# thalesfm/differentiable-renderer

Measured on AMD Instinct MI355X. Metric: Mray/s (fwd+bwd), Cornell 512x512 @64spp depth 8, higher is better.
Workload: dtype f32; 1 GPU; config 3: Cornell 512x512, 64 spp, depth 8, fwd + radiative backprop w.r.t. the albedos; scene 'cornell' (cornell box of render.cpp:26-59) 512x512, 64 spp per GPU, depth 8 (-b 8 -p 1), fwd + radiative-backprop gradients of 4 parameters; program=builtin, parallelism=1 GPU, gpu_max_hw_queues=4 (set by this script before the HIP runtime started)

## Files before the change

differentiable-renderer_amd/csrc/drt_path.h:

```cpp
#pragma once

#include "drt_kernels.h"

#define DRT_DRAW_TABLE (3 * DRT_MAX_DEPTH + 8)

struct PathArgs {
    int32_t W, H, spp;
    int32_t shard, n_shards, band;
    uint32_t Pb, p0, Sb, s0, spr, n_ranges, n_groups;
    int32_t min_bounces, depth_cap, cap_is_roulette, cap_draws;
    uint32_t rr_threshold, seed, rng_stream;
    uint32_t regen_min;
    uint32_t shade_min, descend_min;
    int32_t gimg_param;
    uint32_t gen_rows, gen_clog2;
    uint32_t hist_lds, hist_stride;
    uint32_t gimg_row, pad_gen;
    unsigned long long hist_ovf;
    double p_rr, inv_p_rr;
    double eye[3], fwd[3], right[3], up[3];
    double tan_half, aspect, inv_W, inv_H;
    float p_rr_f, inv_p_rr_f;
    float eye_f[3], fwd_f[3], right_f[3], up_f[3], cs_step_f, ct_step_f;
};
// ... 335 lines not shown
template <typename R>
__device__ inline void gen_zero(GenBlock<R>& gb)
{
    typedef typename GenAcc<R>::T GT;
    for (uint32_t i = threadIdx.x; i < (DRT_BLOCK / DRT_WAVE) * DRT_GEN_TABLE; i += DRT_BLOCK)
        (&gb.table[0][0])[i] = GT(0);
}
template <typename R, int NC, typename SL>
__device__ inline void gen_begin(GenBlock<R>& gb, const SL& lds, const DevScene<R>* __restrict__ sc, const PathArgs& a, uint32_t* hist,
                                 uint32_t* hist_ovf, Tangents<R, DRT_NP_ANY, NC>& tg)
{
    stage_gen(gb.gl, lds, sc);
    tg.gl = &gb.gl;
    tg.hist = hist + threadIdx.x;
    tg.hist_ovf = hist_ovf + (size_t)blockIdx.x * DRT_BLOCK + threadIdx.x;
    tg.gsum = mk<R>(R(0), R(0), R(0));
    tg.gimg_row = a.gimg_row;
    tg.hist_lds = a.hist_lds;
    tg.hist_stride = a.hist_stride;
    tg.clog2 = a.gen_clog2;
    tg.table = &gb.table[threadIdx.x / DRT_WAVE][threadIdx.x & ((1u << a.gen_clog2) - 1u)];
    tg.acc = nullptr;
    tg.new_path();
}
template <typename R>
__device__ inline void gen_finish(const GenBlock<R>& gb, const PathArgs& a, double* __restrict__ gpart)
{
    __syncthreads();
    const uint32_t copies = 1u << a.gen_clog2;
    for (uint32_t r = threadIdx.x; r < a.gen_rows; r += DRT_BLOCK) {
        double v = 0;
        for (int ww = 0; ww < DRT_BLOCK / DRT_WAVE; ++ww)
            for (uint32_t c = 0; c < copies; ++c)
                v += (double)gb.table[ww][(r << a.gen_clog2) + c];
        gpart[(size_t)blockIdx.x * a.gen_rows + r] = v;
    }
}

#define DRT_NC_ROLES(nc, colour_mask, emission_mask) ((int)(nc) | (int)(colour_mask) << 8 | (int)(emission_mask) << 16)
#define DRT_NC_OF(ncr) ((int)(ncr) & 0xFF)
#define DRT_ROLES_OF(ncr) ((int)(ncr) >> 8)
#define DRT_ROLES_CORNELL DRT_ROLES_OF(DRT_NC_ROLES(0, 0x7, 0x8))
template <int NP, int NC, int ROLES>
struct PathRoles {
    static constexpr int all = NP > 0 ? (1 << NP) - 1 : 0;
    static constexpr int colm = ROLES ? (ROLES & 0xFF) & ((1 << NC) - 1) : (1 << NC) - 1;
    static constexpr int emitm = ROLES ? (ROLES >> 8) & all : all;
    static __device__ constexpr bool colour(int p) { return (colm >> p) & 1; }
    static __device__ constexpr bool emission(int p) { return (emitm >> p) & 1; }
    static __device__ constexpr bool only_emission(int p) { return emitm == (1 << p); }
};

template <typename R, int NP, int NC, bool LOSS = false, typename SL = PathSceneLds<R>, int ROLES = 0>
__device__ inline void add_emission(const SL& lds, const TangentLds<R>& tl, const R* __restrict__ params, uint32_t eid, R inv_pk,
                                    V3<R> T, V3<R> g, V3<R>& L, Tangents<R, NP, NC>& tg)
{
    const V3<R> E = load_param<R, (NP != 0)>(lds, params, (int)eid) * inv_pk;
    V3<R> Tr = T;
    if (NC > 0 || NP == DRT_NP_ANY || NP == DRT_NP_TANGENT)
        Tr = mk<R>((tg.zc & 0xFFu) ? R(0) : T.x, (tg.zc & 0xFF00u) ? R(0) : T.y, (tg.zc & 0xFF0000u) ? R(0) : T.z);
    L = L + Tr * E;
    if constexpr (NP == DRT_NP_TANGENT) {
        const R* vd = tg.dl->dir + (eid < DRT_PATH_LDS_PARAMS ? eid : 0u) * 3u;
        const V3<R> Ed = mk<R>(vd[0], vd[1], vd[2]) * inv_pk;
        const V3<R> d0 = mk<R>(fma_r(E.x, tg.S.x, Ed.x), fma_r(E.y, tg.S.y, Ed.y), fma_r(E.z, tg.S.z, Ed.z));
        const V3<R> d1 = E * tg.Z;
        const uint32_t zx = tg.zc & 0xFFu, zy = tg.zc & 0xFF00u, zz = tg.zc & 0xFF0000u;
        tg.dL = mk<R>(fma_r(T.x, zx == 0u ? d0.x : (zx == 0x1u ? d1.x : R(0)), tg.dL.x),
                      fma_r(T.y, zy == 0u ? d0.y : (zy == 0x100u ? d1.y : R(0)), tg.dL.y),
                      fma_r(T.z, zz == 0u ? d0.z : (zz == 0x10000u ? d1.z : R(0)), tg.dL.z));
    } else
    if constexpr (NP == DRT_NP_ANY) {
        if (LOSS)
            g = mk<R>(R(2) * (L.x - g.x), R(2) * (L.y - g.y), R(2) * (L.z - g.z));
        const V3<R> gE = g * E;
        const uint32_t ebits = pid_unpack(tg.gl->invc[eid < DRT_PATH_LDS_PARAMS ? eid : 0][3]);
        if ((ebits & 0xFFFFu) != DRT_SLOT_NONE && eid < DRT_PATH_LDS_PARAMS)
            tg.add(ebits & 0xFFFFu, g * Tr * inv_pk);
        const V3<R> TgE = Tr * gE;
        const V3<R> U = mk<R>((tg.zc & 0xFFu) == 0x1u ? T.x * gE.x : R(0), (tg.zc & 0xFF00u) == 0x100u ? T.y * gE.y : R(0),
                              (tg.zc & 0xFF0000u) == 0x10000u ? T.z * gE.z : R(0));
        const uint32_t nw = tg.nv >> 2;
        for (uint32_t w = 0; wave_any(w < nw); ++w)
            tg.add_word(w < nw ? tg.load_word(w) : 0xFFFFFFFFu, TgE, U);
        tg.add_word(tg.cur, TgE, U);
    } else
    if constexpr (NP > 0) {
        if (NC > 0)
            asm volatile("" ::: "memory");
        if (LOSS)
            g = mk<R>(R(2) * (L.x - g.x), R(2) * (L.y - g.y), R(2) * (L.z - g.z));
        const V3<R> gE = g * E, gT = g * Tr * inv_pk;
#pragma unroll
        for (int p = 0; p < NP; ++p) {
            typedef PathRoles<NP, NC, ROLES> RL;
            const bool is_colour = (RL::colm >> p) & 1, is_emission = (RL::emitm >> p) & 1;
            if (ROLES != 0 && !is_colour && !is_emission)
                continue;
            const bool own = (ROLES != 0 && RL::emitm == (1 << p)) || eid == (uint32_t)p;
            const V3<R> ap = tg.acc_get(p);
            V3<R> a0 = mk<R>(ap.x + (own ? gT.x : R(0)), ap.y + (own ? gT.y : R(0)), ap.z + (own ? gT.z : R(0)));
            if (ROLES != 0 && !is_emission)
                a0 = ap;
            if (is_colour) {
                const uint32_t n = (tg.cnt[p >> 2] >> (8 * (p & 3))) & 0xFFu;
                const R nf = (R)(int)n;
                V3<R> dT = mk<R>(Tr.x * (nf * tl.invc[p][0]), Tr.y * (nf * tl.invc[p][1]), Tr.z * (nf * tl.invc[p][2]));
                const uint32_t zb = __builtin_amdgcn_readfirstlane(tl.inc[p][3]);
                if (zb) {
                    const bool one = n == 1u;
                    if (zb & 1u) dT.x = (one && (tg.zc & 0xFFu) == 0x1u) ? T.x : R(0);
                    if (zb & 2u) dT.y = (one && (tg.zc & 0xFF00u) == 0x100u) ? T.y : R(0);
                    if (zb & 4u) dT.z = (one && (tg.zc & 0xFF0000u) == 0x10000u) ? T.z : R(0);
                }
                tg.acc_set(p, mk<R>(fma_r(dT.x, gE.x, a0.x), fma_r(dT.y, gE.y, a0.y), fma_r(dT.z, gE.z, a0.z)));
            } else
                tg.acc_set(p, a0);
        }
    }
}

template <typename R>
struct CameraLane {
    R cs0, ct0;
};

template <typename R>
struct PathVertex {
    V3<R> P, nrm, d;
    uint32_t ids;
    int material;
    bool hit, scattered;
};

template <typename R, bool SPEC, int NP, int NC, typename SG, bool FREEZE_BY_ROW = false>
__device__ inline void path_bounce(const PathArgs& a, const PathSceneLds<R>& lds, const TangentLds<R>& tl, const DevScene<R>* __restrict__ sc,
                                   const R* __restrict__ params, const ProgRecs<SG::n, R>& recs, uint32_t key,
                                   R pk, R inv_pk, uint32_t n_theta, bool next_rr, bool next_cap, bool live, V3<R> g,
                                   typename Q4<R>::T& ra, typename Q2<R>::T& rb, V3<R>& T, V3<R>& L, Tangents<R, NP, NC>& tg,
                                   bool& alive, bool& capped, bool& on_light, uint32_t& light, PathVertex<R>* vo = nullptr,
                                   bool last = false, const float* __restrict__ seed_px = nullptr, const uint32_t* ih = nullptr)
{
    auto draw = [&](uint32_t n) { return ih ? drt_rng_combine(ih[n], key) : rng_draw(a.rng_stream, key, n); };
    const HitRec<R> h = path_closest_hit<SG>(sc, recs, ra, rb);
    const bool hit = live && h.prim >= 0;
    const int prim = h.prim >= 0 ? h.prim : 0;
    const V3<R> o = mk<R>(ra.x, ra.y, ra.z);
    const V3<R> d = mk<R>(ra.w, rb.x, rb.y);
    const V3<R> P = o + d * h.t;
    const DevShape<R>& sh = lds.sc.shapes[prim];
    const uint32_t ids = (uint32_t)sh.pad;
    const uint32_t cid = ids & 0xFFFFu, eid = ids >> 16;
    const bool has_bxdf = cid != DRT_ID_NONE, emits = hit && eid != DRT_ID_NONE;
    on_light = emits && !has_bxdf;
    light = eid;
    if (last && !vo) {
        if (wave_any(emits && has_bxdf)) {
            if (emits && has_bxdf) {
                if (NP != 0 && seed_px)
                    g = mk<R>((R)seed_px[0], (R)seed_px[1], (R)seed_px[2]);
                add_emission<R, NP, NC>(lds, tl, params, eid, inv_pk, T, g, L, tg);
            }
        }
        alive = false;
        capped = false;
        if (!a.cap_is_roulette) {
            const bool rr_kills = next_rr && draw(n_theta + 2) < a.rr_threshold;
            capped = hit && has_bxdf && !rr_kills;
        }
        return;
    }
    const V3<R> ctr = mk<R>(sh.p[0], sh.p[1], sh.p[2]);
    const V3<R> nsph = normalize(P - ctr);
    const bool is_plane = sh.type == DRT_SHAPE_PLANE;
    V3<R> nrm = mk<R>(is_plane ? ctr.x : nsph.x, is_plane ? ctr.y : nsph.y, is_plane ? ctr.z : nsph.z);
#ifdef DRT_USER_SHAPES
    if (sh.type >= DRT_SHAPE_USER) {
        const R p8[8] = {sh.p[0], sh.p[1], sh.p[2], sh.p[3], lds.user_q[prim][0], lds.user_q[prim][1], lds.user_q[prim][2], lds.user_q[prim][3]};
        nrm = user_normal<R>(sh.type - DRT_SHAPE_USER, p8, P);
    }
#endif
    if (vo) {
        vo->P = P; vo->nrm = nrm; vo->d = d;
        vo->ids = ids;
        vo->material = sh.material;
        vo->hit = hit;
        vo->scattered = hit && has_bxdf;
    }
    if (wave_any(emits && has_bxdf)) {
        if (emits && has_bxdf) {
            if (NP != 0 && seed_px)
                g = mk<R>((R)seed_px[0], (R)seed_px[1], (R)seed_px[2]);
            add_emission<R, NP, NC>(lds, tl, params, eid, inv_pk, T, g, L, tg);
        }
    }
    const DevMaterial<R>& m = lds.sc.materials[has_bxdf ? sh.material : 0];
    V3<R> wo;
    R q, bs;
    sample_bxdf<R, SPEC>(m, nrm, d, draw(n_theta), draw(n_theta + 1), wo, q, bs);
    const R c = dot(nrm, wo);
    const R mk_ = div_r(bs * c, q * pk);
    const bool rr_kills = next_rr && draw(n_theta + 2) < a.rr_threshold;
    alive = hit && has_bxdf && !next_cap && !rr_kills;
    capped = hit && has_bxdf && next_cap && !a.cap_is_roulette && !rr_kills;
    constexpr bool REST = FREEZE_BY_ROW && NC > 0 && NP != DRT_NP_ANY;
    constexpr bool DIR = NP == DRT_NP_TANGENT, BY_ROW = REST || DIR;
    const int cidx = DIR ? (alive ? (int)cid : DRT_PATH_LDS_PARAMS) : (REST ? (alive ? (int)cid : DRT_TANGENT_REST) : (has_bxdf ? (int)cid : 0));
    V3<R> col;
    if constexpr (DIR) {
        const int row = cidx < DRT_PATH_LDS_PARAMS ? cidx : DRT_PATH_LDS_PARAMS;
        const R *rec = tg.dl->colnz[row], *ds = tg.dl->dlog[row], *dz = tg.dl->dzero[row];
        col = mk<R>(rec[0], rec[1], rec[2]);
        tg.zc += pid_unpack(rec[3]);
        tg.S = mk<R>(tg.S.x + ds[0], tg.S.y + ds[1], tg.S.z + ds[2]);
        tg.Z = mk<R>(tg.Z.x + dz[0], tg.Z.y + dz[1], tg.Z.z + dz[2]);
    } else
    if constexpr (NP == DRT_NP_ANY) {
        const R* rec = tg.gl->colnz[cidx < DRT_PATH_LDS_PARAMS ? cidx : 0];
        col = mk<R>(rec[0], rec[1], rec[2]);
        tg.zc += alive ? pid_unpack(rec[3]) : 0u;
        if (ih)
            tg.template push<false>(alive, cid);
        else
            tg.template push<true>(live, alive ? cid : 0xFFu);
    } else
        col = NC > 0 ? mk<R>(tl.colnz[cidx][0], tl.colnz[cidx][1], tl.colnz[cidx][2]) : load_param<R, (NP > 0)>(lds, params, cidx);
    const V3<R> cmv = col * (BY_ROW ? (alive ? mk_ : R(1)) : mk_);
    const V3<R> cm = BY_ROW ? cmv : mk<R>(alive ? cmv.x : R(1), alive ? cmv.y : R(1), alive ? cmv.z : R(1));
    if constexpr (REST) {
        tg.cnt[0] += tl.inc[cidx][0];
        if (NC > 4)
            tg.cnt[NC > 4 ? 1 : 0] += tl.inc[cidx][1];
        tg.zc += tl.inc[cidx][2];
    } else
    if constexpr (NC > 0 && NP != DRT_NP_ANY) {
        tg.cnt[0] += alive ? tl.inc[cidx][0] : 0u;
        if (NC > 4)
            tg.cnt[NC > 4 ? 1 : 0] += alive ? tl.inc[cidx][1] : 0u;
        tg.zc += alive ? tl.inc[cidx][2] : 0u;
    }
    T = T * cm;
    const V3<R> no = P + wo * R(1e-3);
    ra.x = no.x; ra.y = no.y; ra.z = no.z; ra.w = wo.x;
    rb.x = wo.y; rb.y = wo.z;
}

#ifndef DRT_CAMERA_ARGS_F32
#define DRT_CAMERA_ARGS_F32 1
#endif
template <typename R, bool ARGS_F32 = (DRT_CAMERA_ARGS_F32 != 0)>
__device__ inline uint32_t path_camera(const PathArgs& a, const CameraLane<R>& cl, uint32_t gpix, uint32_t px, uint32_t py, uint32_t sl,
                                       typename Q4<R>::T& ra, typename Q2<R>::T& rb)
{
    const uint64_t path = (uint64_t)gpix * (uint64_t)a.spp + (uint64_t)(a.s0 + sl);
    const uint32_t key = (uint32_t)path;
    if (sizeof(R) == 4) {
        const float cs_step = ARGS_F32 ? a.cs_step_f : (float)(2. * a.aspect * a.tan_half * a.inv_W);
        const float ct_step = ARGS_F32 ? a.ct_step_f : (float)(2. * a.tan_half * a.inv_H);
        const V3<float> eye = ARGS_F32 ? mk<float>(a.eye_f[0], a.eye_f[1], a.eye_f[2]) : mk<float>((float)a.eye[0], (float)a.eye[1], (float)a.eye[2]);
        const V3<float> fw = ARGS_F32 ? mk<float>(a.fwd_f[0], a.fwd_f[1], a.fwd_f[2]) : mk<float>((float)a.fwd[0], (float)a.fwd[1], (float)a.fwd[2]);
        const V3<float> rt = ARGS_F32 ? mk<float>(a.right_f[0], a.right_f[1], a.right_f[2]) : mk<float>((float)a.right[0], (float)a.right[1], (float)a.right[2]);
        const V3<float> upv = ARGS_F32 ? mk<float>(a.up_f[0], a.up_f[1], a.up_f[2]) : mk<float>((float)a.up[0], (float)a.up[1], (float)a.up[2]);
        const float cs = fmaf(u01(0.f, rng_draw(a.rng_stream, key, 0)), cs_step, (float)cl.cs0);
        const float ct = fmaf(u01(0.f, rng_draw(a.rng_stream, key, 1)), ct_step, (float)cl.ct0);
        const V3<float> dir = mk<float>(fw.x + cs * rt.x - ct * upv.x, fw.y + cs * rt.y - ct * upv.y, fw.z + cs * rt.z - ct * upv.z);
        const V3<float> dn = normalize(dir);
        ra.x = (R)eye.x; ra.y = (R)eye.y; ra.z = (R)eye.z; ra.w = (R)dn.x;
        rb.x = (R)dn.y; rb.y = (R)dn.z;
    } else {
        const double u1 = (double)rng_draw(a.rng_stream, key, 0) / DRT_RAND_MAX_D;
        const double u2 = (double)rng_draw(a.rng_stream, key, 1) / DRT_RAND_MAX_D;
        const double s = ((double)px + u1) / (double)a.W;
        const double t = ((double)py + u2) / (double)a.H;
        const double cs = (2. * s - 1.) * a.aspect * a.tan_half;
        const double ct = (2. * t - 1.) * a.tan_half;
        double dx = a.fwd[0] + cs * a.right[0] - ct * a.up[0];
        double dy = a.fwd[1] + cs * a.right[1] - ct * a.up[1];
        double dz = a.fwd[2] + cs * a.right[2] - ct * a.up[2];
        const double inv = 1.0 / sqrt(dx * dx + dy * dy + dz * dz);
        ra.x = (R)a.eye[0]; ra.y = (R)a.eye[1]; ra.z = (R)a.eye[2]; ra.w = (R)(dx * inv);
        rb.x = (R)(dy * inv); rb.y = (R)(dz * inv);
    }
    return key;
}
template <typename R>
__device__ inline uint32_t path_camera(const PathArgs& a, const CameraLane<R>& cl, uint32_t gpix, uint32_t sl,
                                       typename Q4<R>::T& ra, typename Q2<R>::T& rb)
{
    uint32_t px = 0, py = 0;
    if (sizeof(R) != 4) {
        py = gpix / (uint32_t)a.W;
        px = gpix - py * (uint32_t)a.W;
    }
    return path_camera<R, false>(a, cl, gpix, px, py, sl, ra, rb);
}

#ifndef DRT_LEAN_MAX_SHAPES
#ifdef DRT_USER_SHAPES
#define DRT_LEAN_MAX_SHAPES (-1)
#else
#define DRT_LEAN_MAX_SHAPES 10
#endif
#endif
template <size_t RB, bool SPEC, int NP, int NSG, bool REGEN>
constexpr int path_min_blocks()
{
    if (NP == DRT_NP_TANGENT)
        return RB == 4 ? (REGEN ? DRT_TANGENT_REGEN_MIN_BLOCKS : DRT_TANGENT_MIN_BLOCKS) : ((REGEN || SPEC) ? 2 : DRT_TANGENT_F64_MIN_BLOCKS);
    if (RB == 4 && NP <= 4) {
        if (!REGEN)
            return SPEC ? ((NP == DRT_NP_ANY || NSG > DRT_LEAN_MAX_SHAPES) ? 5 : DRT_LOCKSTEP_SPEC_MIN_BLOCKS)
                        : (NP == DRT_NP_ANY ? DRT_LOCKSTEP_GEN_MIN_BLOCKS : (NSG <= DRT_LEAN_MAX_SHAPES ? DRT_LOCKSTEP_MIN_BLOCKS : DRT_LOCKSTEP_GEN_MIN_BLOCKS));
        return (NP == DRT_NP_ANY && NSG == 0) ? 4
                                              : (SPEC ? 5 : DRT_REGEN_MIN_BLOCKS);
    }
    return (RB == 8 && NP <= 4 && !REGEN && !SPEC) ? DRT_F64_MIN_BLOCKS : 1;
}

template <typename R, bool SPEC, int NP, int NCR, typename SG, bool REGEN = false, bool LOSS = false>
__global__ void __launch_bounds__(DRT_BLOCK, (path_min_blocks<sizeof(R), SPEC, NP, SG::n, REGEN>()))
k_path(PathArgs a, const DevScene<R>* __restrict__ sc, const R* __restrict__ params, const float* __restrict__ adjoint,
       double* __restrict__ gpart, double* __restrict__ fpart, uint32_t* __restrict__ counts,
       unsigned long long* __restrict__ total, double* __restrict__ gimg_part)
{
    if (total && blockIdx.x == 0 && threadIdx.x < 8)
        total[threadIdx.x] = 0;
    typedef typename Q4<R>::T R4;
    typedef typename Q2<R>::T R2;
    constexpr int NC = DRT_NC_OF(NCR), ROLES = DRT_ROLES_OF(NCR);
    __shared__ PathSceneLds<R> lds;
    __shared__ double s_red[REGEN ? 1 : DRT_BLOCK / DRT_WAVE][DRT_FAST_PARAMS * 3];
    __shared__ TangentLds<R> s_tl;
    constexpr bool GEN = NP == DRT_NP_ANY;
    __shared__ typename PickT<GEN, GenBlock<R>, NoLds>::T s_gen;
    extern __shared__ uint32_t s_hist[];
    constexpr bool DIR = NP == DRT_NP_TANGENT;
    __shared__ typename PickT<DIR, DirLds<R>, NoLds>::T s_dir;
    if constexpr (GEN)
        gen_zero(s_gen);
    stage_path_scene(lds, sc, params);
    const TangentLds<R>& tl = s_tl;
    if (NC > 0 && !GEN)
        stage_tangents(s_tl, lds);

    const uint32_t lane = threadIdx.x & (DRT_WAVE - 1);
    const uint32_t w = grid_wave();
    const uint32_t range = w / a.n_groups, group = w - range * a.n_groups;
    const uint32_t lp = group * DRT_WAVE + lane;
    const bool have = range < a.n_ranges && lp < a.Pb;
    const uint32_t s_begin = range * a.spr;
    const uint32_t s_end = s_begin + a.spr < a.Sb ? s_begin + a.spr : a.Sb;

    Tangents<R, NP, NC> tg;
    __shared__ R s_acc[NP > 0 ? NP * 3 : 1][DRT_BLOCK];
    tg.acc = &s_acc[0][threadIdx.x];
    if constexpr (GEN)
        gen_begin(s_gen, lds, sc, a, s_hist, reinterpret_cast<uint32_t*>(a.hist_ovf), tg);
    else if constexpr (DIR) {
        stage_dir(s_dir, lds, params);
        tg.dl = &s_dir;
        tg.new_path();
    } else {
#pragma unroll
        for (int p = 0; p < NP; ++p)
            tg.acc_set(p, mk<R>(R(0), R(0), R(0)));
    }
    double fx = 0, fy = 0, fz = 0;
    double tx = 0, ty = 0, tz = 0;
    uint32_t n_seg = 0, n_capped = 0;

    uint32_t gpix = 0, px = 0, py = 0;
    V3<R> g = mk<R>(R(1), R(1), R(1));
    if (have) {
        gpix = path_global_pixel(a, a.p0 + lp);
        py = gpix / (uint32_t)a.W;
        px = gpix - py * (uint32_t)a.W;
        if (NP != 0 && adjoint)
            g = mk<R>((R)adjoint[(size_t)gpix * 3], (R)adjoint[(size_t)gpix * 3 + 1], (R)adjoint[(size_t)gpix * 3 + 2]);
    }
    CameraLane<R> cl;
    cl.cs0 = (R)((2. * (double)px * a.inv_W - 1.) * a.aspect * a.tan_half);
    cl.ct0 = (R)((2. * (double)py * a.inv_H - 1.) * a.tan_half);
    constexpr bool ARGS_F32 = sizeof(R) == 4 && !REGEN && DRT_CAMERA_ARGS_F32 != 0 && SG::n <= DRT_LEAN_MAX_SHAPES;
    const R pk_rr = ARGS_F32 ? (R)a.p_rr_f : (R)a.p_rr, inv_p_rr = ARGS_F32 ? (R)a.inv_p_rr_f : (R)a.inv_p_rr;
    ProgRecs<SG::n, R> recs;
    __shared__ typename PickT<(SG::n == 0), ProgLds, NoLds>::T s_prog;
    recs.lds = reinterpret_cast<const ProgLds*>(&s_prog);
    if (SG::n > 0)
        recs.template load<SG>(sc);
    if constexpr (sizeof(R) == 4 && SG::n == 0) {
        const DevScene<float>* scf = reinterpret_cast<const DevScene<float>*>(sc);
        if (threadIdx.x < DRT_PROG_SORTED_MAX) {
            s_prog.rec[threadIdx.x] = *reinterpret_cast<const float4*>(scf->sorted[threadIdx.x]);
            s_prog.shape[threadIdx.x] = scf->sorted_shape[threadIdx.x];
        }
        if (threadIdx.x < 8)
            s_prog.kind_begin[threadIdx.x] = scf->kind_begin[threadIdx.x];
        __syncthreads();
    }

    if (range < a.n_ranges && !REGEN) {
    for (uint32_t sl = s_begin; sl < s_end; ++sl) {
        R4 ra;
        R2 rb;
        const uint32_t key = path_camera<R, ARGS_F32>(a, cl, gpix, px, py, sl, ra, rb);
        bool live = have && a.depth_cap > 0 && !(a.min_bounces <= 0 && rng_draw(a.rng_stream, key, 2) < a.rr_threshold);
        V3<R> T = mk<R>(R(1), R(1), R(1)), L = mk<R>(R(0), R(0), R(0));
        uint32_t end_ids = DRT_ID_NONE;
        R end_inv_pk = R(1);
        if (NC > 0 || GEN || DIR)
            tg.new_path();
        for (int kk = 0; kk < a.depth_cap; ++kk) {
            const uint32_t n_live = (uint32_t)__popcll(wave_ballot(live));
            if (n_live == 0)
                break;
            n_seg += n_live;
            const R pk = kk >= a.min_bounces ? pk_rr : R(1);
            const R inv_pk = kk >= a.min_bounces ? inv_p_rr : R(1);
            const uint32_t n_theta = draw_offset(kk, 0, a.min_bounces) + camera_draw_base(a.min_bounces);
            const bool next_rr = (kk + 1) >= a.min_bounces;
            const bool next_cap = (kk + 1) >= a.depth_cap;
            bool alive, capped, on_light;
            uint32_t light;
            path_bounce<R, SPEC, NP, NC, SG, (DRT_FREEZE_BY_ROW != 0 && sizeof(R) == 4 && !SPEC && SG::n <= DRT_LEAN_MAX_SHAPES)>(a, lds, tl, sc, params, recs, key, pk, inv_pk, n_theta, next_rr, next_cap, live, g,
                                                    ra, rb, T, L, tg, alive, capped, on_light, light, nullptr, next_cap);
            end_ids = on_light ? light : end_ids;
            end_inv_pk = on_light ? inv_pk : end_inv_pk;
            if (next_cap && !a.cap_is_roulette)
                n_capped += (uint32_t)__popcll(wave_ballot(capped));
            live = alive;
        }
        if (wave_any(end_ids != DRT_ID_NONE)) {
            if (end_ids != DRT_ID_NONE)
                add_emission<R, NP, NC, LOSS, PathSceneLds<R>, ROLES>(lds, tl, params, end_ids, end_inv_pk, T, g, L, tg);
        }
        fx += (double)L.x; fy += (double)L.y; fz += (double)L.z;
        if constexpr (DIR) {
            tx += (double)tg.dL.x; ty += (double)tg.dL.y; tz += (double)tg.dL.z;
        }
    }
    }
    __shared__ R s_pcs[REGEN ? DRT_BLOCK : 1], s_pct[REGEN ? DRT_BLOCK : 1];
    __shared__ uint32_t s_pgpix[REGEN ? DRT_BLOCK : 1];
    __shared__ double s_film[REGEN ? 3 : 1][REGEN ? DRT_BLOCK : 1];
    __shared__ uint32_t s_ih[REGEN ? DRT_DRAW_TABLE : 1];
    __shared__ double s_tfilm[REGEN && DIR ? 3 : 1][REGEN && DIR ? DRT_BLOCK : 1];
    if constexpr (REGEN && DIR) {
        s_tfilm[0][threadIdx.x] = 0.0; s_tfilm[1][threadIdx.x] = 0.0; s_tfilm[2][threadIdx.x] = 0.0;
    }
    if (REGEN) {
        for (uint32_t n = threadIdx.x; n < DRT_DRAW_TABLE; n += DRT_BLOCK)
            s_ih[REGEN ? n : 0] = drt_rng_index_hash(a.rng_stream, n);
        s_pcs[threadIdx.x] = cl.cs0;
        s_pct[threadIdx.x] = cl.ct0;
        s_pgpix[threadIdx.x] = have ? gpix : 0xFFFFFFFFu;
        s_film[0][threadIdx.x] = 0.0; s_film[REGEN ? 1 : 0][threadIdx.x] = 0.0; s_film[REGEN ? 2 : 0][threadIdx.x] = 0.0;
        __syncthreads();
    }
    if (range < a.n_ranges && REGEN) {
        const uint32_t wbase = threadIdx.x & ~(uint32_t)(DRT_WAVE - 1);
        const uint32_t n_items = DRT_WAVE * (s_end - s_begin);
        uint32_t n_next = 0;
        uint32_t key = 0, pix = wbase, pgpix = 0;
        int kk = 0;
        bool live = false;
        R4 ra;
        R2 rb;
        ra.x = ra.y = ra.z = ra.w = R(0);
        rb.x = rb.y = R(0);
        V3<R> T = mk<R>(R(1), R(1), R(1)), L = mk<R>(R(0), R(0), R(0));
        if (NC > 0 || GEN || DIR)
            tg.new_path();
        const int first_rr = a.min_bounces > 1 ? a.min_bounces : 1;
        for (;;) {
            const uint64_t idle_mask = wave_ballot(!live);
            const uint32_t n_idle = (uint32_t)__popcll(idle_mask), n_run = DRT_WAVE - n_idle;
            if (n_next < n_items && (n_idle >= a.regen_min || n_idle >= n_run)) {
                const uint32_t n = n_next + __builtin_amdgcn_mbcnt_hi((uint32_t)(idle_mask >> 32), __builtin_amdgcn_mbcnt_lo((uint32_t)idle_mask, 0u));
                if (!live && n < n_items) {
                    pix = wbase + (n & (DRT_WAVE - 1));
                    const uint32_t gp = s_pgpix[pix];
                    if (gp != 0xFFFFFFFFu) {
                        pgpix = gp;
                        CameraLane<R> pc;
                        pc.cs0 = s_pcs[pix];
                        pc.ct0 = s_pct[pix];
                        key = path_camera<R>(a, pc, gp, s_begin + (n >> 6), ra, rb);
                        kk = 0;
                        live = a.depth_cap > 0 && !(a.min_bounces <= 0 && rng_draw(a.rng_stream, key, 2) < a.rr_threshold);
                        T = mk<R>(R(1), R(1), R(1));
                        L = mk<R>(R(0), R(0), R(0));
                        if (NC > 0 || GEN || DIR)
                            tg.new_path();
                    }
                }
                n_next += n_idle < n_items - n_next ? n_idle : n_items - n_next;
            }
            const uint32_t n_live = (uint32_t)__popcll(wave_ballot(live));
            if (n_live == 0) {
                if (n_next >= n_items)
                    break;
                continue;
            }
            n_seg += n_live;
            const bool rr_here = kk >= a.min_bounces;
            const R pk = rr_here ? pk_rr : R(1);
            const R inv_pk = rr_here ? inv_p_rr : R(1);
            const int rr_draws = kk - first_rr + 1;
            const uint32_t n_theta = 2u * (uint32_t)kk + (uint32_t)(rr_draws > 0 ? rr_draws : 0) + camera_draw_base(a.min_bounces);
            const bool next_rr = (kk + 1) >= a.min_bounces;
            const bool next_cap = (kk + 1) >= a.depth_cap;
            bool alive, capped, on_light;
            uint32_t light;
            V3<R> gp3 = mk<R>(R(1), R(1), R(1));
            const float* seed_px = (NP != 0 && adjoint) ? adjoint + (size_t)pgpix * 3 : (const float*)nullptr;
            path_bounce<R, SPEC, NP, NC, SG>(a, lds, tl, sc, params, recs, key, pk, inv_pk, n_theta, next_rr, next_cap, live, gp3,
                                                    ra, rb, T, L, tg, alive, capped, on_light, light, nullptr, false, seed_px, s_ih);
            if (!a.cap_is_roulette)
                n_capped += (uint32_t)__popcll(wave_ballot(capped));
            const bool ended = live && !alive;
            if (wave_any(ended)) {
                if (ended) {
                    if (on_light) {
                        if (seed_px)
                            gp3 = mk<R>((R)seed_px[0], (R)seed_px[1], (R)seed_px[2]);
                        add_emission<R, NP, NC, LOSS>(lds, tl, params, light, inv_pk, T, gp3, L, tg);
                    }
                    if (L.x != R(0) || L.y != R(0) || L.z != R(0)) {
                        atomicAdd(&s_film[0][pix], (double)L.x);
                        atomicAdd(&s_film[REGEN ? 1 : 0][pix], (double)L.y);
                        atomicAdd(&s_film[REGEN ? 2 : 0][pix], (double)L.z);
                    }
                    if constexpr (REGEN && DIR) {
                        if (tg.dL.x != R(0) || tg.dL.y != R(0) || tg.dL.z != R(0)) {
                            atomicAdd(&s_tfilm[0][pix], (double)tg.dL.x);
                            atomicAdd(&s_tfilm[1][pix], (double)tg.dL.y);
                            atomicAdd(&s_tfilm[2][pix], (double)tg.dL.z);
                        }
                    }
                }
            }
            live = alive;
            ++kk;
        }
    }
    if (REGEN) {
        __syncthreads();
        fx = s_film[0][threadIdx.x]; fy = s_film[REGEN ? 1 : 0][threadIdx.x]; fz = s_film[REGEN ? 2 : 0][threadIdx.x];
        if constexpr (REGEN && DIR) {
            tx = s_tfilm[0][threadIdx.x]; ty = s_tfilm[1][threadIdx.x]; tz = s_tfilm[2][threadIdx.x];
        }
    }

    if (range < a.n_ranges) {
        if (fpart && have) {
            double* f = fpart + ((size_t)range * 3) * a.Pb + lp;
            f[0] = fx; f[(size_t)a.Pb] = fy; f[(size_t)a.Pb * 2] = fz;
        }
        if constexpr (GEN && NC == 1) if (gimg_part && have) {
            double* f = gimg_part + ((size_t)range * 3) * a.Pb + lp;
            f[0] = (double)tg.gsum.x; f[(size_t)a.Pb] = (double)tg.gsum.y; f[(size_t)a.Pb * 2] = (double)tg.gsum.z;
        }
        if constexpr (DIR) if (gimg_part && have) {
            double* f = gimg_part + ((size_t)range * 3) * a.Pb + lp;
            f[0] = tx; f[(size_t)a.Pb] = ty; f[(size_t)a.Pb * 2] = tz;
        }
        if constexpr (NP > 0) if (gimg_part && have) {
            const V3<R> v = tg.acc_get(a.gimg_param > 0 && a.gimg_param < NP ? a.gimg_param : 0);
            double* f = gimg_part + ((size_t)range * 3) * a.Pb + lp;
            f[0] = (double)v.x; f[(size_t)a.Pb] = (double)v.y; f[(size_t)a.Pb * 2] = (double)v.z;
        }
        if (lane == 0) {
            counts[w] = n_seg;
            counts[(size_t)a.n_groups * a.n_ranges + w] = n_capped;
        }
    }
    if constexpr (GEN)
        gen_finish(s_gen, a, gpart);
    else
    if (NP > 0) {
        const int wv = threadIdx.x / DRT_WAVE;
        double (*red)[DRT_FAST_PARAMS * 3] = s_red;
        if (REGEN) {
            __syncthreads();
            red = reinterpret_cast<double (*)[DRT_FAST_PARAMS * 3]>(&s_film[0][0]);
        }
#pragma unroll
        for (int r = 0; r < NP * 3; ++r) {
            double v = (double)tg.acc[r * DRT_BLOCK];
#pragma unroll
            for (int o2 = DRT_WAVE / 2; o2 > 0; o2 >>= 1)
                v += __shfl_down(v, o2);
            if (lane == 0)
                red[wv][r] = v;
        }
        __syncthreads();
        if (threadIdx.x < DRT_FAST_PARAMS * 3) {
            double v = 0;
            if ((int)threadIdx.x < NP * 3)
                for (int ww = 0; ww < DRT_BLOCK / DRT_WAVE; ++ww)
                    v += red[ww][threadIdx.x];
            gpart[(size_t)blockIdx.x * (DRT_FAST_PARAMS * 3) + threadIdx.x] = v;
        }
    }
}

template <typename R, bool SPEC, typename SG>
__device__ inline void unbiased_walk(const PathArgs& a, const PathSceneLds<R>& lds, const TangentLds<R>& tl, const DevScene<R>* __restrict__ sc,
                                     const R* __restrict__ params, const ProgRecs<SG::n, R>& recs, uint32_t key,
                                     R pk_rr, R inv_p_rr, bool live, typename Q4<R>::T ra, typename Q2<R>::T rb, int kk,
                                     uint32_t& nd, uint32_t& n_seg, uint32_t& n_capped, V3<R>& L, PathVertex<R>& first, bool& any_vertex)
{
    V3<R> T = mk<R>(R(1), R(1), R(1));
    L = mk<R>(R(0), R(0), R(0));
    any_vertex = false;
    Tangents<R, 0, 0> none;
    const V3<R> g1 = mk<R>(R(1), R(1), R(1));
    for (;;) {
        const uint32_t n_live = (uint32_t)__popcll(wave_ballot(live));
        if (n_live == 0)
            break;
        n_seg += n_live;
        const bool rr_here = kk >= a.min_bounces;
        const R pk = rr_here ? pk_rr : R(1), inv_pk = rr_here ? inv_p_rr : R(1);
        const bool next_rr = (kk + 1) >= a.min_bounces, next_cap = (kk + 1) >= a.depth_cap;
        bool alive, capped, on_light;
        uint32_t light;
        PathVertex<R> v;
        path_bounce<R, SPEC, 0, 0, SG>(a, lds, tl, sc, params, recs, key, pk, inv_pk, nd, next_rr, next_cap, live, g1, ra, rb, T, L,
                                              none, alive, capped, on_light, light, &v);
        const uint32_t rr_drawn = (next_rr && (!next_cap || a.cap_draws)) ? 1u : 0u;
        if (live) {
            if (!any_vertex && v.hit) {
                first = v;
                any_vertex = true;
            }
            nd += v.scattered ? 2u + rr_drawn : (v.hit ? rr_drawn : 0u);
        }
        if (wave_any(live && on_light)) {
            if (live && on_light)
                add_emission<R, 0, 0>(lds, tl, params, light, inv_pk, T, g1, L, none);
        }
        if (!a.cap_is_roulette)
            n_capped += (uint32_t)__popcll(wave_ballot(live && capped));
        live = alive;
        ++kk;
    }
}

#ifndef DRT_UNBIASED_MIN_BLOCKS
#define DRT_UNBIASED_MIN_BLOCKS 4
#endif
template <typename R, bool SPEC, int NP, typename SG>
__global__ void __launch_bounds__(DRT_BLOCK, (sizeof(R) == 4 ? DRT_UNBIASED_MIN_BLOCKS : 1))
k_path_unbiased(PathArgs a, const DevScene<R>* __restrict__ sc, const R* __restrict__ params, const float* __restrict__ adjoint,
                double* __restrict__ gpart, double* __restrict__ fpart, uint32_t* __restrict__ counts,
                unsigned long long* __restrict__ total)
{
    if (total && blockIdx.x == 0 && threadIdx.x < 8)
        total[threadIdx.x] = 0;
    typedef typename Q4<R>::T R4;
    typedef typename Q2<R>::T R2;
    __shared__ PathSceneLds<R> lds;
    __shared__ double s_red[DRT_BLOCK / DRT_WAVE][DRT_FAST_PARAMS * 3];
    constexpr bool GEN = NP == DRT_NP_ANY;
    __shared__ typename PickT<GEN, GenBlock<R>, NoLds>::T s_gen;
    if constexpr (GEN)
        gen_zero(s_gen);
    stage_path_scene(lds, sc, params);
    const TangentLds<R>& tl = *reinterpret_cast<const TangentLds<R>*>(&lds);
    Tangents<R, GEN ? DRT_NP_ANY : 0, 0> gt;
    if constexpr (GEN)
        gen_begin(s_gen, lds, sc, a, (uint32_t*)nullptr, (uint32_t*)nullptr, gt);

    const uint32_t lane = threadIdx.x & (DRT_WAVE - 1);
    const uint32_t w = grid_wave();
    const uint32_t range = w / a.n_groups, group = w - range * a.n_groups;
    const uint32_t lp = group * DRT_WAVE + lane;
    const bool have = range < a.n_ranges && lp < a.Pb;
    const uint32_t s_begin = range * a.spr;
    const uint32_t s_end = s_begin + a.spr < a.Sb ? s_begin + a.spr : a.Sb;

    V3<R> acc[NP > 0 ? NP : 1];
#pragma unroll
    for (int p = 0; p < NP; ++p)
        acc[p] = mk<R>(R(0), R(0), R(0));
    double fx = 0, fy = 0, fz = 0;
    uint32_t n_seg = 0, n_capped = 0;
    uint32_t gpix = 0, px = 0, py = 0;
    V3<R> g0 = mk<R>(R(1), R(1), R(1));
    if (have) {
        gpix = path_global_pixel(a, a.p0 + lp);
        py = gpix / (uint32_t)a.W;
        px = gpix - py * (uint32_t)a.W;
        if (adjoint)
            g0 = mk<R>((R)adjoint[(size_t)gpix * 3], (R)adjoint[(size_t)gpix * 3 + 1], (R)adjoint[(size_t)gpix * 3 + 2]);
    }
    CameraLane<R> cl;
    cl.cs0 = (R)((2. * (double)px * a.inv_W - 1.) * a.aspect * a.tan_half);
    cl.ct0 = (R)((2. * (double)py * a.inv_H - 1.) * a.tan_half);
    constexpr bool ARGS_F32 = sizeof(R) == 4 && DRT_CAMERA_ARGS_F32 != 0 && SG::n <= DRT_LEAN_MAX_SHAPES;
    const R pk_rr = ARGS_F32 ? (R)a.p_rr_f : (R)a.p_rr, inv_p_rr = ARGS_F32 ? (R)a.inv_p_rr_f : (R)a.inv_p_rr;
    ProgRecs<SG::n, R> recs;
    __shared__ ProgLds s_prog;
    recs.lds = &s_prog;
    if (SG::n > 0)
        recs.template load<SG>(sc);
    if (sizeof(R) == 4 && SG::n == 0) {
        const DevScene<float>* scf = reinterpret_cast<const DevScene<float>*>(sc);
        if (threadIdx.x < DRT_PROG_SORTED_MAX) {
            s_prog.rec[threadIdx.x] = *reinterpret_cast<const float4*>(scf->sorted[threadIdx.x]);
            s_prog.shape[threadIdx.x] = scf->sorted_shape[threadIdx.x];
        }
        if (threadIdx.x < 8)
            s_prog.kind_begin[threadIdx.x] = scf->kind_begin[threadIdx.x];
        __syncthreads();
    }
    auto rr_drawn = [&](int d) { return d >= a.min_bounces && (d < a.depth_cap || a.cap_draws != 0); };

    if (range < a.n_ranges) {
        for (uint32_t sl = s_begin; sl < s_end; ++sl) {
            R4 ra;
            R2 rb;
            const uint32_t key = path_camera<R, ARGS_F32>(a, cl, gpix, px, py, sl, ra, rb);
            uint32_t nd = 2;
            bool live = have && a.depth_cap > 0;
            if (rr_drawn(0)) {
                live = live && !(rng_draw(a.rng_stream, key, nd) < a.rr_threshold);
                ++nd;
            }
            V3<R> L0;
            PathVertex<R> cur;
            bool in_chain;
            unbiased_walk<R, SPEC, SG>(a, lds, tl, sc, params, recs, key, pk_rr, inv_p_rr, live, ra, rb, 0, nd, n_seg, n_capped, L0,
                                              cur, in_chain);
            fx += (double)L0.x; fy += (double)L0.y; fz += (double)L0.z;
            in_chain = in_chain && have;
            int cdepth = 0;
            V3<R> g = g0;
            while (wave_any(in_chain)) {
                V3<R> gq = mk<R>(R(0), R(0), R(0)), fcol = gq;
                R bs = R(0);
                bool go = false;
                R4 sa = ra;
                R2 sb = rb;
                uint32_t cid = DRT_ID_NONE;
                if (in_chain) {
                    const R inv_pk = cdepth >= a.min_bounces ? inv_p_rr : R(1);
                    const V3<R> g1 = g * inv_pk;
                    const uint32_t eid = cur.ids >> 16;
                    cid = cur.ids & 0xFFFFu;
                    if constexpr (GEN) {
                        if (eid < DRT_PATH_LDS_PARAMS) {
                            const uint32_t row = pid_unpack(gt.gl->invc[eid][3]) & 0xFFFFu;
                            if (row != DRT_SLOT_NONE)
                                gt.add(row, g1);
                        }
                    }
#pragma unroll
                    for (int p = 0; p < NP; ++p) {
                        const bool own = eid == (uint32_t)p;
                        acc[p] = mk<R>(acc[p].x + (own ? g1.x : R(0)), acc[p].y + (own ? g1.y : R(0)), acc[p].z + (own ? g1.z : R(0)));
                    }
                    if (cid == DRT_ID_NONE) {
                        in_chain = false;
                    } else {
                        const DevMaterial<R>& m = lds.sc.materials[cur.material];
                        V3<R> wo;
                        R q;
                        sample_bxdf<R, SPEC>(m, cur.nrm, cur.d, rng_draw(a.rng_stream, key, nd), rng_draw(a.rng_stream, key, nd + 1), wo, q, bs);
                        nd += 2;
                        const R c = dot(cur.nrm, wo);
                        gq = g1 * div_r(c, q);
                        fcol = load_param<R, true>(lds, params, (int)cid) * bs;
                        go = (cdepth + 1) < a.depth_cap;
                        if (rr_drawn(cdepth + 1)) {
                            go = go && !(rng_draw(a.rng_stream, key, nd) < a.rr_threshold);
                            ++nd;
                        }
                        const V3<R> no = cur.P + wo * R(1e-3);
                        sa.x = no.x; sa.y = no.y; sa.z = no.z; sa.w = wo.x;
                        sb.x = wo.y; sb.y = wo.z;
                    }
                }
                V3<R> Ls;
                PathVertex<R> nxt;
                bool any_vertex;
                unbiased_walk<R, SPEC, SG>(a, lds, tl, sc, params, recs, key, pk_rr, inv_p_rr, in_chain && go, sa, sb, cdepth + 1, nd,
                                                  n_seg, n_capped, Ls, nxt, any_vertex);
                if (in_chain) {
                    const V3<R> df = Ls * gq * bs;
                    if constexpr (GEN) {
                        if (cid < DRT_PATH_LDS_PARAMS) {
                            const uint32_t row = pid_unpack(gt.gl->invc[cid][3]) & 0xFFFFu;
                            if (row != DRT_SLOT_NONE)
                                gt.add(row, df);
                        }
                    }
#pragma unroll
                    for (int p = 0; p < NP; ++p) {
                        const bool own = cid == (uint32_t)p;
                        acc[p] = mk<R>(acc[p].x + (own ? df.x : R(0)), acc[p].y + (own ? df.y : R(0)), acc[p].z + (own ? df.z : R(0)));
                    }
                    if (!any_vertex) {
                        in_chain = false;
                    } else {
                        g = fcol * gq;
                        cur = nxt;
                        ++cdepth;
                    }
                }
            }
        }
        if (fpart && have) {
            double* f = fpart + ((size_t)range * 3) * a.Pb + lp;
            f[0] = fx; f[(size_t)a.Pb] = fy; f[(size_t)a.Pb * 2] = fz;
        }
        if (lane == 0) {
            counts[w] = n_seg;
            counts[(size_t)a.n_groups * a.n_ranges + w] = n_capped;
        }
    }
    if constexpr (GEN)
        gen_finish(s_gen, a, gpart);
    else
    {
        const int wv = threadIdx.x / DRT_WAVE;
#pragma unroll
        for (int r = 0; r < NP * 3; ++r) {
            const V3<R> v3 = acc[r / 3];
            double v = (double)(r % 3 == 0 ? v3.x : (r % 3 == 1 ? v3.y : v3.z));
#pragma unroll
            for (int o2 = DRT_WAVE / 2; o2 > 0; o2 >>= 1)
                v += __shfl_down(v, o2);
            if (lane == 0)
                s_red[wv][r] = v;
        }
        __syncthreads();
        if (threadIdx.x < DRT_FAST_PARAMS * 3) {
            double v = 0;
            if ((int)threadIdx.x < NP * 3)
                for (int ww = 0; ww < DRT_BLOCK / DRT_WAVE; ++ww)
                    v += s_red[ww][threadIdx.x];
            gpart[(size_t)blockIdx.x * (DRT_FAST_PARAMS * 3) + threadIdx.x] = v;
        }
    }
}

__global__ void __launch_bounds__(DRT_BLOCK)
k_film_parts(const double* __restrict__ fpart, uint32_t n_ranges, uint32_t Pb, uint32_t p0, double* __restrict__ film)
{
    const uint32_t stride = gridDim.x * blockDim.x;
    for (uint32_t j = blockIdx.x * blockDim.x + threadIdx.x; j < Pb; j += stride) {
        double r = 0, g = 0, b = 0;
        for (uint32_t q = 0; q < n_ranges; ++q) {
            const double* f = fpart + ((size_t)q * 3) * Pb + j;
            r += f[0]; g += f[(size_t)Pb]; b += f[(size_t)Pb * 2];
        }
        double* f = film + (size_t)(p0 + j) * 3;
        f[0] += r; f[1] += g; f[2] += b;
    }
}

__global__ void __launch_bounds__(DRT_BLOCK)
k_path_finish(PathArgs a, const double* __restrict__ fpart, float* __restrict__ out, uint32_t film_blocks,
              const double* __restrict__ gpart, int n_blocks, int n_rows, int row_stride, double* __restrict__ grad, uint32_t grad_words,
              const uint32_t* __restrict__ counts, uint32_t n_waves, unsigned long long* __restrict__ total, uint32_t count_rows = 2,
              const unsigned short* __restrict__ slot_map = nullptr)
{
    __shared__ double red[DRT_BLOCK];
    if (blockIdx.x < film_blocks) {
        const uint32_t stride = film_blocks * DRT_BLOCK;
        const double inv = 1.0 / (double)a.spp;
        for (uint32_t j = blockIdx.x * DRT_BLOCK + threadIdx.x; j < a.Pb; j += stride) {
            double r = 0, g = 0, b = 0;
            for (uint32_t q = 0; q < a.n_ranges; ++q) {
                const double* f = fpart + ((size_t)q * 3) * a.Pb + j;
                r += f[0]; g += f[(size_t)a.Pb]; b += f[(size_t)a.Pb * 2];
            }
            const uint32_t gp = path_global_pixel(a, a.p0 + j);
            drt_f3 px;
            px.x = (float)(r * inv); px.y = (float)(g * inv); px.z = (float)(b * inv);
            *reinterpret_cast<drt_f3_u*>(out + (size_t)gp * 3) = px;
        }
        return;
    }
    if (blockIdx.x < film_blocks + grad_words) {
        const int p = (int)(blockIdx.x - film_blocks);
        int src = p;
        if (slot_map) {
            const int slot = slot_map[p / 3];
            src = slot == (int)DRT_SLOT_NONE ? n_rows : slot * 3 + p % 3;
        }
        double v = 0;
        if (src < n_rows)
            for (int b = threadIdx.x; b < n_blocks; b += DRT_BLOCK)
                v += gpart[(size_t)b * row_stride + src];
// ... 33 lines not shown
```

Measured before the change: 202,500 Mray/s.

## Compute wave pixel coords cheaply, reload tail args from kernarg, reduce gradients via LDS columns

For the lean f32 gradient kernel, pixel coordinates are derived once per wave from a base index plus lane with a carry, which avoids a per-lane integer divide. Output pointers and sizes are reloaded from the kernarg segment after the path loop, so they need not stay live in registers. The per-parameter shuffle reduction becomes a column reduction in which each group of four lanes sums one accumulator row from LDS, replacing many shuffle rounds. Together these aim to cut register pressure and tail overhead, at the cost of relying on the kernarg struct layout matching the kernel signature.

```diff
diff --git a/differentiable-renderer_amd/csrc/drt_path.h b/differentiable-renderer_amd/csrc/drt_path.h
--- a/differentiable-renderer_amd/csrc/drt_path.h
+++ b/differentiable-renderer_amd/csrc/drt_path.h
@@ -661,6 +661,56 @@
 #define DRT_LEAN_MAX_SHAPES 10
 #endif
 #endif
+#ifndef DRT_WAVE_PIXEL
+#define DRT_WAVE_PIXEL 1
+#endif
+#ifndef DRT_LDS_REDUCE
+#define DRT_LDS_REDUCE 1
+#endif
+#ifndef DRT_TAIL_ARGS
+#define DRT_TAIL_ARGS 1
+#endif
+template <typename R>
+struct PathKernArgs {
+    PathArgs a;
+    const DevScene<R>* sc;
+    const R* params;
+    const float* adjoint;
+    double *gpart, *fpart;
+    uint32_t* counts;
+    unsigned long long* total;
+    double* gimg_part;
+};
+template <typename R, bool SPEC, int NP, int NSG, bool REGEN>
+constexpr bool path_lean_form()
+{
+    return sizeof(R) == 4 && !SPEC && !REGEN && NP > 0 && NP <= 4 && NSG <= DRT_LEAN_MAX_SHAPES;
+}
+
+template <typename R, int ROWS>
+__device__ inline double path_reduce_columns(const R* col0, uint32_t lane, int& row)
+{
+    static_assert(ROWS * 4 <= DRT_WAVE, "a lane per (row, l)");
+    __builtin_amdgcn_fence(__ATOMIC_ACQ_REL, "wavefront");
+    __builtin_amdgcn_wave_barrier();
+    row = (int)(lane >> 2);
+    const R* c = col0 + (row < ROWS ? row : 0) * DRT_BLOCK + (lane & 3u);
+    double v[16];
+#pragma unroll
+    for (int k = 0; k < 16; ++k)
+        v[k] = (double)c[4 * k];
+#pragma unroll
+    for (int k = 0; k < 8; ++k) v[k] += v[k + 8];
+#pragma unroll
+    for (int k = 0; k < 4; ++k) v[k] += v[k + 4];
+#pragma unroll
+    for (int k = 0; k < 2; ++k) v[k] += v[k + 2];
+    double s = v[0] + v[1];
+    s += __shfl_down(s, 2);
+    s += __shfl_down(s, 1);
+    return s;
+}
+
 template <size_t RB, bool SPEC, int NP, int NSG, bool REGEN>
 constexpr int path_min_blocks()
 {
@@ -730,10 +780,32 @@
 
     uint32_t gpix = 0, px = 0, py = 0;
     V3<R> g = mk<R>(R(1), R(1), R(1));
+    constexpr bool LEAN = path_lean_form<R, SPEC, NP, SG::n, REGEN>();
     if (have) {
-        gpix = path_global_pixel(a, a.p0 + lp);
-        py = gpix / (uint32_t)a.W;
-        px = gpix - py * (uint32_t)a.W;
+        if constexpr (LEAN && DRT_WAVE_PIXEL != 0) {
+            const uint32_t W = (uint32_t)a.W, base = a.p0 + group * DRT_WAVE;
+            uint32_t ly = base / W;
+            px = base - ly * W + lane;
+            if (W >= DRT_WAVE) {
+                const bool carry = px >= W;
+                px -= carry ? W : 0u;
+                ly += carry ? 1u : 0u;
+            } else {
+                const uint32_t q = px / W;
+                px -= q * W;
+                ly += q;
+            }
+            py = ly;
+            if (a.n_shards > 1) {
+                const uint32_t b = ly / (uint32_t)a.band, r = ly - b * (uint32_t)a.band;
+                py = (b * (uint32_t)a.n_shards + (uint32_t)a.shard) * (uint32_t)a.band + r;
+            }
+            gpix = py * W + px;
+        } else {
+            gpix = path_global_pixel(a, a.p0 + lp);
+            py = gpix / (uint32_t)a.W;
+            px = gpix - py * (uint32_t)a.W;
+        }
         if (NP != 0 && adjoint)
             g = mk<R>((R)adjoint[(size_t)gpix * 3], (R)adjoint[(size_t)gpix * 3 + 1], (R)adjoint[(size_t)gpix * 3 + 2]);
     }
@@ -911,6 +983,13 @@
         }
     }
 
+    if constexpr (LEAN && DRT_TAIL_ARGS != 0) {
+        typedef const __attribute__((address_space(4))) PathKernArgs<R> KA;
+        KA* ka = (KA*)__builtin_amdgcn_kernarg_segment_ptr();
+        asm volatile("" : "+s"(ka));
+        a.Pb = ka->a.Pb; a.n_groups = ka->a.n_groups; a.n_ranges = ka->a.n_ranges; a.gimg_param = ka->a.gimg_param;
+        gpart = ka->gpart; fpart = ka->fpart; counts = ka->counts; gimg_part = ka->gimg_part;
+    }
     if (range < a.n_ranges) {
         if (fpart && have) {
             double* f = fpart + ((size_t)range * 3) * a.Pb + lp;
@@ -944,6 +1023,12 @@
             __syncthreads();
             red = reinterpret_cast<double (*)[DRT_FAST_PARAMS * 3]>(&s_film[0][0]);
         }
+        if constexpr (LEAN && DRT_LDS_REDUCE != 0) {
+            int row;
+            const double v = path_reduce_columns<R, (NP > 0 ? NP * 3 : 1)>(&s_acc[0][wv * DRT_WAVE], lane, row);
+            if ((lane & 3u) == 0 && row < NP * 3)
+                red[wv][row] = v;
+        } else {
 #pragma unroll
         for (int r = 0; r < NP * 3; ++r) {
             double v = (double)tg.acc[r * DRT_BLOCK];
@@ -952,6 +1037,7 @@
                 v += __shfl_down(v, o2);
             if (lane == 0)
                 red[wv][r] = v;
+        }
         }
         __syncthreads();
         if (threadIdx.x < DRT_FAST_PARAMS * 3) {
```

New measurement: 204,300 Mray/s (median of 6 runs). About the same (+0.9%).
